# sebrahimi1988/dss-ml-at-scale

Measured on AMD Instinct MI355X. Metric: samples/sec, higher is better.
Workload: dtype bf16; 1 GPU; model=resnet18, global_batch=212, parallelism=dp1+hipgraph

## Files before the change

### mi355x_scale/ops/csrc/bindings.cpp

```cpp

#include <torch/extension.h>
#include <ATen/hip/HIPContext.h>
#include <hip/hip_runtime.h>

extern "C" void launch_normalize_u8_to_bf16(
    const uint8_t* in, void* out, const float* scale_dev,
    const float* shift_dev, long long n, hipStream_t stream);

void normalize_u8_to_bf16(torch::Tensor in, torch::Tensor out,
                          torch::Tensor scale, torch::Tensor shift) {
  TORCH_CHECK(in.is_cuda() && out.is_cuda(), "tensors must be on GPU");
  TORCH_CHECK(in.scalar_type() == torch::kUInt8, "input must be uint8");
  TORCH_CHECK(out.scalar_type() == torch::kBFloat16, "output must be bf16");
  TORCH_CHECK(in.is_contiguous(), "input must be contiguous (NHWC)");
  TORCH_CHECK(in.numel() == out.numel(), "element count mismatch");
  TORCH_CHECK(scale.is_cuda() && shift.is_cuda() && scale.numel() == 3 &&
                  shift.numel() == 3,
              "scale/shift must be 3-element device float tensors");
  TORCH_CHECK(scale.scalar_type() == torch::kFloat32 &&
              shift.scalar_type() == torch::kFloat32,
              "scale/shift must be float32");
  auto stream = at::cuda::getCurrentHIPStream();
  launch_normalize_u8_to_bf16(
      in.data_ptr<uint8_t>(), out.data_ptr(),
      scale.data_ptr<float>(), shift.data_ptr<float>(),
      (long long)in.numel(), stream.stream());
}

extern "C" void launch_groupfit_eval(
    const float* yT, const float* xc0, const float* xc1, const float* xc2,
    const float* pj0, const float* pj1, const float* pj2, const int* orders,
    float* mse, unsigned char* statusv,
    const float* b0, const float* b1, const float* b2,
    const float* w0, const float* w1, const float* w2,
    int T, long long G, int S, int C,
    int KX, hipStream_t stream);

extern "C" void launch_diff_center(const float* yT, float* wc, float* wm,
                                   int T, long long G, int S, int d,
                                   hipStream_t stream);

extern "C" void launch_exog_project_mfma(const float* P, const float* wc,
                                         float* beta, int n, long long G,
                                         int KX, hipStream_t stream);

extern "C" void launch_groupfit_final(
    const float* yT, const float* xc0, const float* xc1, const float* xc2,
    const float* pj0, const float* pj1, const float* pj2,
    const int* best_order, float* fitted, float* params,
    unsigned char* statusv,
    const float* b0, const float* b1, const float* b2,
    const float* w0, const float* w1, const float* w2,
    int T, long long G, int KX, hipStream_t stream);

extern "C" void launch_stem_conv_fwd(const void* x, const void* w, void* out,
                                     void* wp_scratch, float* partial,
                                     int Nb, int H, int W, int HO, int WO,
                                     hipStream_t stream, int phase_mask);
extern "C" int stem_fwd_stat_blocks(int Nb, int HO);
extern "C" void launch_stem_conv_wrw(const void* x, const void* dy,
                                     float* dw_f32, void* dw_bf16,
                                     int Nb, int H, int W, int HO, int WO,
                                     hipStream_t stream, int phase_mask);
extern "C" void launch_conv3x3_wrw(const void* x, const void* dy,
                                   float* part, void* dw_bf16,
                                   int Nb, int H, int W, int C,
                                   int chunks, hipStream_t stream,
                                   int phase_mask);
extern "C" int conv3x3_wrw_chunks(int Nb, int H, int C, int chunks_req);

static void _check_f32(const torch::Tensor& t, const char* name) {
  TORCH_CHECK(t.is_cuda() && t.scalar_type() == torch::kFloat32 &&
                  t.is_contiguous(),
              name, " must be contiguous f32 on GPU");
}

void groupfit_eval(torch::Tensor yT, torch::Tensor xc0, torch::Tensor xc1,
                   torch::Tensor xc2, torch::Tensor pj0, torch::Tensor pj1,
                   torch::Tensor pj2, torch::Tensor orders,
                   torch::Tensor mse, torch::Tensor status, int64_t S,
                   torch::Tensor b0, torch::Tensor b1, torch::Tensor b2,
                   torch::Tensor w0, torch::Tensor w1, torch::Tensor w2) {
  _check_f32(yT, "yT"); _check_f32(xc0, "xc0"); _check_f32(xc1, "xc1");
  _check_f32(xc2, "xc2"); _check_f32(pj0, "pj0"); _check_f32(pj1, "pj1");
  _check_f32(pj2, "pj2"); _check_f32(mse, "mse");
  TORCH_CHECK(orders.scalar_type() == torch::kInt32 && orders.is_cuda());
  TORCH_CHECK(status.scalar_type() == torch::kUInt8 && status.is_cuda());
  int T = yT.size(0);
  long long G = yT.size(1);
  int C = orders.size(0);
  TORCH_CHECK(S > 8 && S <= T, "need 8 < S <= T");
  TORCH_CHECK(mse.size(0) == C && mse.size(1) == G);
  auto stream = at::cuda::getCurrentHIPStream();
  auto fp = [](torch::Tensor& t) -> const float* {
    return t.numel() ? t.data_ptr<float>() : nullptr;
  };
  launch_groupfit_eval(
      yT.data_ptr<float>(), xc0.data_ptr<float>(), xc1.data_ptr<float>(),
      xc2.data_ptr<float>(), pj0.data_ptr<float>(), pj1.data_ptr<float>(),
      pj2.data_ptr<float>(), orders.data_ptr<int>(), mse.data_ptr<float>(),
      status.data_ptr<uint8_t>(),
      fp(b0), fp(b1), fp(b2), fp(w0), fp(w1), fp(w2),
      T, G, (int)S, C, (int)xc0.size(1),
      stream.stream());
}

void groupfit_final(torch::Tensor yT, torch::Tensor xc0, torch::Tensor xc1,
                    torch::Tensor xc2, torch::Tensor pj0, torch::Tensor pj1,
                    torch::Tensor pj2, torch::Tensor best_order,
                    torch::Tensor fitted, torch::Tensor params,
                    torch::Tensor status,
                    torch::Tensor b0, torch::Tensor b1, torch::Tensor b2,
                    torch::Tensor w0, torch::Tensor w1, torch::Tensor w2) {
  _check_f32(yT, "yT"); _check_f32(fitted, "fitted");
  _check_f32(params, "params");
  TORCH_CHECK(best_order.scalar_type() == torch::kInt32 &&
              best_order.is_cuda());
  int T = yT.size(0);
  long long G = yT.size(1);
  TORCH_CHECK(fitted.size(0) == T && fitted.size(1) == G);
  auto stream = at::cuda::getCurrentHIPStream();
  auto fp = [](torch::Tensor& t) -> const float* {
    return t.numel() ? t.data_ptr<float>() : nullptr;
  };
  launch_groupfit_final(
      yT.data_ptr<float>(), xc0.data_ptr<float>(), xc1.data_ptr<float>(),
      xc2.data_ptr<float>(), pj0.data_ptr<float>(), pj1.data_ptr<float>(),
      pj2.data_ptr<float>(), best_order.data_ptr<int>(),
      fitted.data_ptr<float>(), params.data_ptr<float>(),
      status.data_ptr<uint8_t>(),
      fp(b0), fp(b1), fp(b2), fp(w0), fp(w1), fp(w2),
      T, G, (int)xc0.size(1), stream.stream());
}

void diff_center(torch::Tensor yT, torch::Tensor wc, torch::Tensor wm,
                 int64_t S, int64_t d) {
  _check_f32(yT, "yT"); _check_f32(wc, "wc"); _check_f32(wm, "wm");
  auto stream = at::cuda::getCurrentHIPStream();
  launch_diff_center(yT.data_ptr<float>(), wc.data_ptr<float>(),
                     wm.data_ptr<float>(), yT.size(0), yT.size(1),
                     (int)S, (int)d, stream.stream());
}

void exog_project_mfma(torch::Tensor P, torch::Tensor wc,
                       torch::Tensor beta) {
  _check_f32(P, "P"); _check_f32(wc, "wc"); _check_f32(beta, "beta");
  TORCH_CHECK(P.size(1) == wc.size(0), "K mismatch");
  TORCH_CHECK(beta.size(0) == P.size(0) && beta.size(1) == wc.size(1));
  TORCH_CHECK(P.size(0) <= 16, "KX must fit one MFMA row tile");
  auto stream = at::cuda::getCurrentHIPStream();
  launch_exog_project_mfma(P.data_ptr<float>(), wc.data_ptr<float>(),
                           beta.data_ptr<float>(), P.size(1), wc.size(1),
                           P.size(0), stream.stream());
}


extern "C" int bn_reduce_blocks(long long rows, int C);
extern "C" void launch_bn_fwd_reduce(const void* x, float* partial,
                                     int nblocks, long long rows, int C,
                                     hipStream_t stream);
extern "C" void launch_bn_fwd_finalize(const float* partial, int nblocks,
                                       float* mean, float* invstd,
                                       float* running_mean,
                                       float* running_var, float momentum,
                                       float eps, long long rows, int C,
                                       int update_running,
                                       long long* num_batches_tracked,
                                       hipStream_t stream);
extern "C" void launch_bn_pool_bwd_reduce(
    const void* dp, const unsigned char* code, const void* x,
    const float* mean, const float* invstd, const float* weight,
    const float* bias, float* partial, int nblocks, int N, int H, int W,
    int Ho, int Wo, int C, hipStream_t stream);
extern "C" void launch_bn_pool_bwd_apply(
    const void* dp, const unsigned char* code, const void* x,
    const float* mean, const float* invstd, const float* bias,
    const float* k, void* dx, int N, int H, int W, int Ho, int Wo, int C,
    hipStream_t stream);
extern "C" void launch_bn_fwd_apply(const void* x, const void* res, void* y,
                                    const float* mean, const float* invstd,
                                    const float* weight, const float* bias,
                                    long long rows, int C, int relu,
                                    hipStream_t stream);
extern "C" void launch_bn_bwd_reduce(const void* dz, const void* y,
                                     const void* x, const float* mean,
                                     const float* invstd, float* partial,
                                     void* dym, int nblocks, long long rows,
                                     int C, int relu, hipStream_t stream);
extern "C" void launch_bn_bwd_reduce_join(const void* dz1, const void* dz2,
                                          const void* y, const void* x,
                                          const float* mean,
                                          const float* invstd,
                                          float* partial, void* dym,
                                          int nblocks, long long rows, int C,
                                          int relu, hipStream_t stream);
extern "C" void launch_bn_bwd_reduce_rm(const void* dz, const void* x,
                                        const float* mean,
                                        const float* invstd,
                                        const float* weight,
                                        const float* bias, float* partial,
                                        void* dym, int nblocks,
                                        long long rows, int C,
                                        hipStream_t stream);
extern "C" void launch_bn_bwd_apply_rm(const void* dz, const void* x,
                                       const float* mean,
                                       const float* invstd,
                                       const float* bias, const float* k,
                                       void* dx, long long rows, int C,
                                       hipStream_t stream);
extern "C" void launch_bn_bwd_apply_dym(const void* dym, const void* x,
                                        const float* mean,
                                        const float* invstd, const float* k,
                                        void* dx, long long rows, int C,
                                        hipStream_t stream);
extern "C" void launch_bn_bwd_finalize(const float* partial, int nblocks,
                                       const float* invstd,
// ... 322 lines not shown
  TORCH_CHECK(x.dim() == 4 && dp.dim() == 4, "x and dp must be 4-d");
  TORCH_CHECK(x.is_contiguous(at::MemoryFormat::ChannelsLast) &&
                  dp.is_contiguous(at::MemoryFormat::ChannelsLast),
              "x and dp must be channels_last");
  _PoolGeom g{(int)x.size(0), (int)x.size(1), (int)x.size(2),
              (int)x.size(3), (int)dp.size(2), (int)dp.size(3)};
  TORCH_CHECK(g.C % 8 == 0 && 256 % (g.C / 8) == 0, "bad C");
  TORCH_CHECK(dp.size(0) == g.N && dp.size(1) == g.C, "dp N/C mismatch");
  TORCH_CHECK(g.Ho == (g.H + 1) / 2 && g.Wo == (g.W + 1) / 2,
              "3x3 s2 p1 shape");
  TORCH_CHECK(code.numel() == dp.numel(), "code/dp size mismatch");
  TORCH_CHECK((int64_t)g.N * g.Ho * g.Wo < (int64_t(1) << 31),
              "N*Ho*Wo must be < 2^31");
  return g;
}

torch::Tensor bn_pool_bwd_reduce(torch::Tensor dp, torch::Tensor code,
                                 torch::Tensor x, torch::Tensor mean,
                                 torch::Tensor invstd, torch::Tensor weight,
                                 torch::Tensor bias) {
  _PoolGeom g = _check_bn_pool_bwd(dp, code, x);
  _check_f32(mean, "mean"); _check_f32(invstd, "invstd");
  _check_f32(weight, "weight"); _check_f32(bias, "bias");
  TORCH_CHECK(mean.numel() == g.C && invstd.numel() == g.C &&
                  weight.numel() == g.C && bias.numel() == g.C,
              "channel vectors must be [C]");
  int nb = bn_reduce_blocks((long long)g.N * g.Ho * g.Wo, g.C);
  auto partial = torch::empty(
      {(int64_t)nb * 2 * g.C},
      torch::TensorOptions().dtype(torch::kFloat32).device(x.device()));
  launch_bn_pool_bwd_reduce(dp.data_ptr(), code.data_ptr<uint8_t>(),
                            x.data_ptr(), mean.data_ptr<float>(),
                            invstd.data_ptr<float>(),
                            weight.data_ptr<float>(),
                            bias.data_ptr<float>(),
                            partial.data_ptr<float>(), nb, g.N, g.H, g.W,
                            g.Ho, g.Wo, g.C,
                            at::cuda::getCurrentHIPStream().stream());
  return partial;
}

void bn_pool_bwd_apply(torch::Tensor dp, torch::Tensor code, torch::Tensor x,
                       torch::Tensor mean, torch::Tensor invstd,
                       torch::Tensor bias, torch::Tensor k,
                       torch::Tensor dx) {
  _PoolGeom g = _check_bn_pool_bwd(dp, code, x);
  _check_bn_act(dx, "dx");
  _check_f32(mean, "mean"); _check_f32(invstd, "invstd");
  _check_f32(bias, "bias"); _check_f32(k, "k");
  TORCH_CHECK(mean.numel() == g.C && invstd.numel() == g.C &&
                  bias.numel() == g.C && k.numel() == 3 * g.C,
              "channel vectors must be [C], k [3C]");
  TORCH_CHECK(dx.sizes() == x.sizes() &&
                  dx.is_contiguous(at::MemoryFormat::ChannelsLast),
              "dx must match x (channels_last)");
  launch_bn_pool_bwd_apply(dp.data_ptr(), code.data_ptr<uint8_t>(),
                           x.data_ptr(), mean.data_ptr<float>(),
                           invstd.data_ptr<float>(), bias.data_ptr<float>(),
                           k.data_ptr<float>(), dx.data_ptr(), g.N, g.H,
                           g.W, g.Ho, g.Wo, g.C,
                           at::cuda::getCurrentHIPStream().stream());
}

extern "C" void launch_adam_step(float* p, const float* g, float* m,
                                 float* v, int* step, float lr, float beta1,
                                 float beta2, float eps, float weight_decay,
                                 long long n, hipStream_t stream);

void adam_step(torch::Tensor p, torch::Tensor g, torch::Tensor m,
               torch::Tensor v, torch::Tensor step, double lr, double beta1,
               double beta2, double eps, double weight_decay) {
  _check_f32(p, "p"); _check_f32(g, "g"); _check_f32(m, "m");
  _check_f32(v, "v");
  TORCH_CHECK(step.is_cuda() && step.scalar_type() == torch::kInt32 &&
                  step.numel() == 1,
              "step must be a 1-element int32 device tensor");
  long long n = p.numel();
  TORCH_CHECK(g.numel() == n && m.numel() == n && v.numel() == n,
              "flat buffer length mismatch");
  launch_adam_step(p.data_ptr<float>(), g.data_ptr<float>(),
                   m.data_ptr<float>(), v.data_ptr<float>(),
                   step.data_ptr<int>(), (float)lr, (float)beta1,
                   (float)beta2, (float)eps, (float)weight_decay, n,
                   at::cuda::getCurrentHIPStream().stream());
}

extern "C" void launch_adam_step_mixed(float* master, const void* gb,
                                       const float* gf, float* m, float* v,
                                       void* pb, int* step, float lr,
                                       float beta1, float beta2, float eps,
                                       float weight_decay, long long nb,
                                       long long n, hipStream_t stream);

void adam_step_mixed(torch::Tensor master, torch::Tensor gb,
                     torch::Tensor gf, torch::Tensor m, torch::Tensor v,
                     torch::Tensor pb, torch::Tensor step, double lr,
                     double beta1, double beta2, double eps,
                     double weight_decay) {
  _check_f32(master, "master"); _check_f32(m, "m"); _check_f32(v, "v");
  TORCH_CHECK(gb.scalar_type() == torch::kBFloat16 &&
              pb.scalar_type() == torch::kBFloat16, "gb/pb must be bf16");
  TORCH_CHECK(step.is_cuda() && step.scalar_type() == torch::kInt32 &&
              step.numel() == 1, "step must be int32[1] on device");
  long long n = master.numel();
  long long nb = gb.numel();
  TORCH_CHECK(pb.numel() == nb && gf.numel() == n - nb &&
              m.numel() == n && v.numel() == n, "buffer length mismatch");
  const float* gf_p = gf.numel() ? gf.data_ptr<float>() : nullptr;
  launch_adam_step_mixed(master.data_ptr<float>(), gb.data_ptr(), gf_p,
                         m.data_ptr<float>(), v.data_ptr<float>(),
                         pb.data_ptr(), step.data_ptr<int>(), (float)lr,
                         (float)beta1, (float)beta2, (float)eps,
                         (float)weight_decay, nb, n,
                         at::cuda::getCurrentHIPStream().stream());
}

int64_t stem_fwd_blocks(int64_t Nb, int64_t HO) {
  return stem_fwd_stat_blocks((int)Nb, (int)HO);
}

void stem_conv_fwd(torch::Tensor x, torch::Tensor w, torch::Tensor out,
                   torch::Tensor wp_scratch, int64_t phase_mask = 7,
                   c10::optional<torch::Tensor> partial = c10::nullopt) {
  TORCH_CHECK(x.is_cuda() && x.scalar_type() == torch::kBFloat16);
  TORCH_CHECK(w.is_cuda() && w.scalar_type() == torch::kBFloat16);
  TORCH_CHECK(out.is_cuda() && out.scalar_type() == torch::kBFloat16);
  int Nb = x.size(0), H = x.size(1), W = x.size(2);
  TORCH_CHECK(x.size(3) == 3 && out.size(3) == 64, "stem is 3->64");
  int HO = out.size(1), WO = out.size(2);
  TORCH_CHECK(WO <= 128, "stem kernel handles output rows up to 128 px");
  TORCH_CHECK(w.numel() == 64 * 7 * 7 * 3);
  TORCH_CHECK(wp_scratch.scalar_type() == torch::kBFloat16 &&
              wp_scratch.numel() == 64 * 160);
  TORCH_CHECK(x.is_contiguous() && out.is_contiguous() &&
                  out.size(0) == Nb && HO == (H - 1) / 2 + 1 &&
                  WO == (W - 1) / 2 + 1,
              "stem conv: dense NHWC x/out with 7x7 s2 p3 geometry");
  float* partial_p = nullptr;
  if (partial.has_value()) {
    const torch::Tensor& p = *partial;
    TORCH_CHECK(p.is_cuda() && p.scalar_type() == torch::kFloat32 &&
                    p.is_contiguous() &&
                    p.numel() == 2 * 64 * stem_fwd_blocks(Nb, HO),
                "partial must be fp32 [2*64*stem_fwd_blocks(N, HO)]");
    partial_p = p.data_ptr<float>();
  }
  launch_stem_conv_fwd(x.data_ptr(), w.data_ptr(), out.data_ptr(),
                       wp_scratch.data_ptr(), partial_p,
                       Nb, H, W, HO, WO,
                       at::cuda::getCurrentHIPStream().stream(),
                       (int)phase_mask);
}

void stem_conv_wrw(torch::Tensor x, torch::Tensor dy, torch::Tensor dw_f32,
                   torch::Tensor dw, int64_t phase_mask = 7) {
  TORCH_CHECK(x.is_cuda() && x.scalar_type() == torch::kBFloat16);
  TORCH_CHECK(dy.is_cuda() && dy.scalar_type() == torch::kBFloat16);
  TORCH_CHECK(dw_f32.scalar_type() == torch::kFloat32 &&
              dw_f32.numel() == 64 * 160);
  TORCH_CHECK(dw.scalar_type() == torch::kBFloat16 &&
              dw.numel() == 64 * 7 * 7 * 3);
  int Nb = x.size(0), H = x.size(1), W = x.size(2);
  int HO = dy.size(1), WO = dy.size(2);
  launch_stem_conv_wrw(x.data_ptr(), dy.data_ptr(),
                       dw_f32.data_ptr<float>(), dw.data_ptr(),
                       Nb, H, W, HO, WO,
                       at::cuda::getCurrentHIPStream().stream(),
                       (int)phase_mask);
}

void conv3x3_wrw(torch::Tensor x, torch::Tensor dy, torch::Tensor part,
                 torch::Tensor dw, int64_t phase_mask = 7,
                 int64_t chunks = 0) {
  TORCH_CHECK(x.is_cuda() && x.scalar_type() == torch::kBFloat16);
  TORCH_CHECK(dy.is_cuda() && dy.scalar_type() == torch::kBFloat16);
  int Nb = x.size(0), H = x.size(1), W = x.size(2), C = x.size(3);
  TORCH_CHECK(dy.size(1) == H && dy.size(2) == W && dy.size(3) == C,
              "same-shape 3x3 s1 conv only");
  TORCH_CHECK(C % 64 == 0 && C <= 2048, "C must be a multiple of 64");
  TORCH_CHECK(W >= 3 && W <= 64, "row length outside kernel bounds");
  const int nch = conv3x3_wrw_chunks(Nb, H, C, (int)chunks);
  TORCH_CHECK(part.scalar_type() == torch::kFloat32 &&
              part.numel() >= (long long)nch * C * 9 * C,
              "partial buffer too small for ", nch, " chunks");
  TORCH_CHECK(dw.scalar_type() == torch::kBFloat16 &&
              dw.numel() == (long long)C * 9 * C);
  launch_conv3x3_wrw(x.data_ptr(), dy.data_ptr(), part.data_ptr<float>(),
                     dw.data_ptr(), Nb, H, W, C, nch,
                     at::cuda::getCurrentHIPStream().stream(),
                     (int)phase_mask);
}

int64_t conv3x3_wrw_nchunks(int64_t Nb, int64_t H, int64_t C,
                            int64_t chunks) {
  return conv3x3_wrw_chunks((int)Nb, (int)H, (int)C, (int)chunks);
}

PYBIND11_MODULE(TORCH_EXTENSION_NAME, m) {
  m.def("conv3x3_wrw", &conv3x3_wrw,
        "MFMA 3x3/s1 CxC weight grad (fp32 accum, bf16 cast to view)",
        pybind11::arg("x"), pybind11::arg("dy"), pybind11::arg("part"),
        pybind11::arg("dw"), pybind11::arg("phase_mask") = 7,
        pybind11::arg("chunks") = 0);
  m.def("conv3x3_wrw_nchunks", &conv3x3_wrw_nchunks,
        "partial-buffer chunk count the wrw launcher will use");
  m.def("stem_conv_fwd", &stem_conv_fwd,
        "MFMA stem conv fwd (7x7 s2, 3->64, NHWC bf16)",
        pybind11::arg("x"), pybind11::arg("w"), pybind11::arg("out"),
        pybind11::arg("wp_scratch"), pybind11::arg("phase_mask") = 7,
        pybind11::arg("partial") = pybind11::none());
  m.def("stem_fwd_blocks", &stem_fwd_blocks,
        "block (= BN partial slot) count of the fused-statistics stem fwd");
  m.def("stem_conv_wrw", &stem_conv_wrw,
        "MFMA stem conv weight-grad (fp32 accum + bf16 cast)",
        pybind11::arg("x"), pybind11::arg("dy"), pybind11::arg("dw_f32"),
        pybind11::arg("dw"), pybind11::arg("phase_mask") = 7);
  m.def("normalize_u8_to_bf16", &normalize_u8_to_bf16,
        "fused uint8 NHWC -> normalized bf16 (same memory order)");
  m.def("groupfit_eval", &groupfit_eval,
        "batched per-group ARIMAX candidate evaluation (validation MSE)");
  m.def("groupfit_final", &groupfit_final,
        "batched per-group final fit (fitted values + params)");
  m.def("diff_center", &diff_center,
        "difference + per-group centering of the time-major panel");
  m.def("exog_project_mfma", &exog_project_mfma,
        "design-matrix GEMM beta = P @ Wc on f32 MFMA");
  m.def("bn_fwd_reduce", &bn_fwd_reduce);
  m.def("bn_fwd_finalize", &bn_fwd_finalize,
        "mean/invstd + running stats (+ optional int64 step counter)",
        pybind11::arg("partial"), pybind11::arg("mean"),
        pybind11::arg("invstd"), pybind11::arg("running_mean"),
        pybind11::arg("running_var"), pybind11::arg("momentum"),
        pybind11::arg("eps"), pybind11::arg("rows"), pybind11::arg("C"),
        pybind11::arg("update_running"),
        pybind11::arg("num_batches_tracked") = pybind11::none());
  m.def("bn_fwd_apply", &bn_fwd_apply);
  m.def("bn_bwd_reduce", &bn_bwd_reduce);
  m.def("bn_bwd_reduce_join", &bn_bwd_reduce_join);
  m.def("bn_bwd_reduce_rm", &bn_bwd_reduce_rm);
  m.def("bn_bwd_apply_rm", &bn_bwd_apply_rm);
  m.def("bn_bwd_finalize", &bn_bwd_finalize);
  m.def("bn_bwd_apply", &bn_bwd_apply);
  m.def("bn_bwd_apply_dym", &bn_bwd_apply_dym);
  m.def("adam_step", &adam_step,
        "fused flat Adam step (one kernel over p/g/m/v)");
  m.def("maxpool3x3s2_fwd", &maxpool3x3s2_fwd);
  m.def("bn_maxpool3x3s2_fwd", &bn_maxpool3x3s2_fwd);
  m.def("maxpool3x3s2_bwd", &maxpool3x3s2_bwd);
  m.def("bn_pool_bwd_reduce", &bn_pool_bwd_reduce,
        "stem BN bwd reduce with the max-unpool rebuilt in registers");
  m.def("bn_pool_bwd_apply", &bn_pool_bwd_apply,
        "stem BN bwd apply with the max-unpool rebuilt in registers");
  m.def("adam_step_mixed", &adam_step_mixed,
        "fused flat Adam with bf16 params/grads + fp32 master");
  m.def("arma_generate", &arma_generate,
        "batched ARMA(p,q) sample paths, one group per lane");
}
```

### mi355x_scale/ops/csrc/stemconv.hip

```cpp
#include <hip/hip_runtime.h>
#include <hip/hip_bf16.h>

#define KH 7
#define KW 7
#define CI 3
#define CO 64
#define KTAP (KH * KW * CI)
#define KPAD 160
#define KLDS 168
#define PXPAD 128
#define XTROW ((4 + 2 * PXPAD + KW + 4) * CI + 3)
#define XTOFF 12
#define STRIDE 2
#define PADDING 3

typedef __bf16 bf16;
typedef __attribute__((ext_vector_type(8))) __bf16 bf16x8;
typedef __attribute__((ext_vector_type(4))) __bf16 bf16x4;
typedef __attribute__((ext_vector_type(4))) float f32x4;

__device__ __forceinline__ void stage_band(
    const bf16* __restrict__ x, bf16* xt, int n, int ho, int H, int W,
    int tid, int nthreads, bool prime) {
  const int rowlen = W * CI;
// ... 201 lines not shown
          if (ih >= 0 && ih < H && c >= 0 && c < nch)
            v[u] = reinterpret_cast<const bf16x4*>(
                x + ((long long)n * H + ih) * rowlen)[c];
        }
      }
#pragma unroll
      for (int u = 0; u < STAGE_DEPTH; ++u) {
        const int i = base + tid + u * nthreads;
        if (i < total) reinterpret_cast<bf16x4*>(xt)[i] = v[u];
      }
    }
  } else {
    const int total = nrows_in * XTROW;
    for (int i = tid; i < total; i += nthreads) {
      const int r = i / XTROW, e = i - r * XTROW - XTOFF;
      const int ih = ih0 + r;
      bf16 v = (bf16)0.0f;
      if (ih >= 0 && ih < H && e >= 0 && e < rowlen)
        v = x[((long long)n * H + ih) * rowlen + e];
      xt[i] = v;
    }
  }
}

extern "C" __global__ __launch_bounds__(256, 3) void stem_conv_fwd_stats_kernel(
    const bf16* __restrict__ x,
    const bf16* __restrict__ wp,
    bf16* __restrict__ out,
    float* __restrict__ partial,
    int Nb, int H, int W, int HO, int WO, int nchunks, int phase_mask) {
  __shared__ __attribute__((aligned(16))) bf16 xt[FWD_BAND_ROWS * XTROW];
  __shared__ __attribute__((aligned(16))) bf16 ot[4 * 32 * OTROW];
  __shared__ __attribute__((aligned(16))) unsigned short ktab[4 * KPAD / 4];
  const int tid = threadIdx.x;
  const int wave = tid >> 6;
  const int lane = tid & 63;
  const int row16 = lane & 15;
  const int kgrp = lane >> 4;
  const int n = blockIdx.x / nchunks;
  const int ho0 = (blockIdx.x - n * nchunks) * FWD_ROWS;
  const int rows = min(FWD_ROWS, HO - ho0);

  bf16x8 bfrag[KPAD / 32][4];
#pragma unroll
  for (int kk = 0; kk < KPAD / 32; ++kk)
#pragma unroll
    for (int c = 0; c < 4; ++c)
      bfrag[kk][c] = *reinterpret_cast<const bf16x8*>(
          wp + (c * 16 + row16) * KPAD + kk * 32 + kgrp * 8);

  if (tid < 4 * KPAD / 4) {
    const int g = tid / (KPAD / 4), i = tid - g * (KPAD / 4);
    const int k = (i >> 3) * 32 + g * 8 + (i & 7);
    ktab[tid] = (unsigned short)(2 * koff_of(min(k, KTAP - 1)));
  }
  if (phase_mask & 1)
    stage_band_rows(x, xt, n, ho0 * STRIDE - PADDING,
                    rows * STRIDE + KH - STRIDE, H, W, tid, 256);
  __syncthreads();
  if (!(phase_mask & 4)) return;

  float ssum[4] = {0.f, 0.f, 0.f, 0.f}, ssq[4] = {0.f, 0.f, 0.f, 0.f};
  const int pxb0 = (wave * 32 + row16) * (STRIDE * CI);
  const int pxb1 = (wave * 32 + 16 + row16) * (STRIDE * CI);
  bf16* tw = ot + wave * 32 * OTROW;
#pragma unroll 1
  for (int rr = 0; rr < rows; ++rr) {
    const int rshift = rr * STRIDE * XTROW;
#pragma unroll 1
    for (int m = 0; m < 2; ++m) {
      f32x4 acc[4];
#pragma unroll
      for (int c = 0; c < 4; ++c) acc[c] = (f32x4)0.0f;
      const unsigned rb = 2u * (unsigned)(rshift + (m ? pxb1 : pxb0));
      const uint4* tp = reinterpret_cast<const uint4*>(ktab) + kgrp * 5;
      asm volatile("" : "+v"(tp));
#pragma unroll
      for (int kk = 0; kk < KPAD / 32; ++kk) {
        const uint4 t4 = tp[kk];
        const unsigned tk[4] = {t4.x, t4.y, t4.z, t4.w};
        bf16x8 f;
#pragma unroll
        for (int j = 0; j < 8; ++j) {
          const int k = kk * 32 + kgrp * 8 + j;
          const bool kz = (kk == KPAD / 32 - 1) && k >= KTAP;
          const unsigned pk = tk[j >> 1];
          const unsigned ob = ((j & 1) ? (pk >> 16) : (pk & 0xffffu)) + rb;
          f[j] = *reinterpret_cast<const bf16*>(
              reinterpret_cast<const char*>(xt) + (kz ? 0u : ob));
        }
#pragma unroll
        for (int c = 0; c < 4; ++c)
          acc[c] = __builtin_amdgcn_mfma_f32_16x16x32_bf16(
              f, bfrag[kk][c], acc[c], 0, 0, 0);
      }
#pragma unroll
      for (int r = 0; r < 4; ++r) {
        const int pxl = m * 16 + kgrp * 4 + r;
        const bool live = wave * 32 + pxl < WO;
#pragma unroll
        for (int c = 0; c < 4; ++c) {
          const bf16 v = (bf16)acc[c][r];
          tw[pxl * OTROW + c * 16 + row16] = v;
          const float f = live ? (float)v : 0.f;
          ssum[c] += f;
          ssq[c] += f * f;
        }
      }
    }
    __builtin_amdgcn_fence(__ATOMIC_RELEASE, "wavefront");
    __builtin_amdgcn_wave_barrier();
    __builtin_amdgcn_fence(__ATOMIC_ACQUIRE, "wavefront");
    const long long rowbase = ((long long)n * HO + ho0 + rr) * WO;
#pragma unroll
    for (int t = 0; t < 4; ++t) {
      const int v = lane + t * 64;
      const int pxl = v >> 3, j8 = (v & 7) * 8;
      const int px = wave * 32 + pxl;
      const bf16x8 val = *reinterpret_cast<const bf16x8*>(
          tw + pxl * OTROW + j8);
      if (px < WO)
        *reinterpret_cast<bf16x8*>(out + (rowbase + px) * CO + j8) = val;
    }
    __builtin_amdgcn_fence(__ATOMIC_RELEASE, "wavefront");
    __builtin_amdgcn_wave_barrier();
    __builtin_amdgcn_fence(__ATOMIC_ACQUIRE, "wavefront");
  }

#pragma unroll
  for (int c = 0; c < 4; ++c) {
    ssum[c] += __shfl_xor(ssum[c], 16, 64);
    ssum[c] += __shfl_xor(ssum[c], 32, 64);
    ssq[c] += __shfl_xor(ssq[c], 16, 64);
    ssq[c] += __shfl_xor(ssq[c], 32, 64);
  }
  float* red = reinterpret_cast<float*>(tw);
  if (kgrp == 0) {
#pragma unroll
    for (int c = 0; c < 4; ++c) {
      red[c * 16 + row16] = ssum[c];
      red[CO + c * 16 + row16] = ssq[c];
    }
  }
  __syncthreads();
  if (tid < 2 * CO) {
    float t = 0.f;
#pragma unroll
    for (int w = 0; w < 4; ++w)
      t += reinterpret_cast<const float*>(ot + w * 32 * OTROW)[tid];
    partial[(long long)tid * gridDim.x + blockIdx.x] = t;
  }
}

extern "C" __global__ __launch_bounds__(256) void stem_conv_wrw_kernel(
    const bf16* __restrict__ x,
    const bf16* __restrict__ dy,
    float* __restrict__ dw,
    int Nb, int H, int W, int HO, int WO, int rows_per_block,
    int phase_mask) {
  __shared__ bf16 xt[8 * XTROW];
  __shared__ bf16 Dy[2 * PXPAD * CO];
  const int tid = threadIdx.x;
  const int wave = tid >> 6;
  const int lane = tid & 63;
  const int row16 = lane & 15;
  const int kgrp = lane >> 4;
  const int nrows = Nb * HO;
  const int mw = (wave >> 1) * 2;
  const int cw = (wave & 1) * 5;
  const int row_limit = min((blockIdx.x + 1) * rows_per_block, nrows);
  const int nch = (WO * CO) >> 3;
  const bf16x8 zv = {(bf16)0.0f, (bf16)0.0f, (bf16)0.0f, (bf16)0.0f,
                     (bf16)0.0f, (bf16)0.0f, (bf16)0.0f, (bf16)0.0f};

  f32x4 acc[2][5];
#pragma unroll
  for (int m = 0; m < 2; ++m)
#pragma unroll
    for (int c = 0; c < 5; ++c) acc[m][c] = (f32x4)0.0f;

  int cur = 0;
  {
    const int row0 = blockIdx.x * rows_per_block;
    if (row0 < nrows) {
      const bf16x8* src = reinterpret_cast<const bf16x8*>(
          dy + (long long)row0 * WO * CO);
      bf16x8* d8 = reinterpret_cast<bf16x8*>(Dy);
      bf16x8 v[4];
#pragma unroll
      for (int u = 0; u < 4; ++u) {
        const int i = tid + u * 256;
        v[u] = (i < nch) ? src[i] : zv;
      }
#pragma unroll
      for (int u = 0; u < 4; ++u) d8[tid + u * 256] = v[u];
    }
  }

  for (int rr = 0; rr < rows_per_block; ++rr) {
    const int row = blockIdx.x * rows_per_block + rr;
    if (row >= nrows) break;
    const int n = row / HO;
    const int ho = row - n * HO;
    const bool prime = (rr == 0) || (ho == 0);
    __syncthreads();
    if (prime)
      for (int i = tid; i < 8 * XTROW; i += 256) xt[i] = (bf16)0.0f;
    __syncthreads();
    if (phase_mask & 1)
      stage_band_ring(x, xt, n, ho, H, W, tid, 256, prime);
    bf16x8 v[4];
    const bool have_next = (phase_mask & 2) && row + 1 < row_limit;
    if (have_next) {
      const bf16x8* src = reinterpret_cast<const bf16x8*>(
          dy + (long long)(row + 1) * WO * CO);
#pragma unroll
      for (int u = 0; u < 4; ++u) {
        const int i = tid + u * 256;
        v[u] = (i < nch) ? src[i] : zv;
      }
    }
    __syncthreads();
    if (phase_mask & 4) {
    } else {
      if (have_next) {
        bf16x8* d8 = reinterpret_cast<bf16x8*>(Dy + (cur ^ 1) * PXPAD * CO);
#pragma unroll
        for (int u = 0; u < 4; ++u) d8[tid + u * 256] = v[u];
        cur ^= 1;
      }
      continue;
    }

#pragma unroll
    for (int sl = 0; sl < 4; ++sl) {
      const int pxbase = sl * 32;
      bf16x8 afrag[2];
#pragma unroll
      for (int m = 0; m < 2; ++m) {
        bf16x8 f;
        const bf16* dycur = Dy + cur * PXPAD * CO;
#pragma unroll
        for (int j = 0; j < 8; ++j)
          f[j] = dycur[(pxbase + kgrp * 8 + j) * CO + (mw + m) * 16 + row16];
        afrag[m] = f;
      }
#pragma unroll
      for (int c = 0; c < 5; ++c) {
        const int k = (cw + c) * 16 + row16;
        const int kh = k / (KW * CI);
        const int r21 = k - kh * (KW * CI);
        const int ko = ((ho * STRIDE - PADDING + kh) & 7) * XTROW +
                       (XTOFF - PADDING * CI) + r21;
        const bool kz = k >= KTAP;
        bf16x8 bfr;
#pragma unroll
        for (int j = 0; j < 8; ++j)
          bfr[j] = kz ? (bf16)0.0f
                      : xt[ko + (pxbase + kgrp * 8 + j) * (STRIDE * CI)];
#pragma unroll
        for (int m = 0; m < 2; ++m)
          acc[m][c] = __builtin_amdgcn_mfma_f32_16x16x32_bf16(
              afrag[m], bfr, acc[m][c], 0, 0, 0);
      }
    }
    if (have_next) {
      bf16x8* d8 = reinterpret_cast<bf16x8*>(Dy + (cur ^ 1) * PXPAD * CO);
#pragma unroll
      for (int u = 0; u < 4; ++u) d8[tid + u * 256] = v[u];
      cur ^= 1;
    }
  }

#pragma unroll
  for (int m = 0; m < 2; ++m)
#pragma unroll
    for (int c = 0; c < 5; ++c)
#pragma unroll
      for (int r = 0; r < 4; ++r) {
        const int co = (mw + m) * 16 + kgrp * 4 + r;
        const int k = (cw + c) * 16 + row16;
        atomicAdd(&dw[co * KPAD + k], acc[m][c][r]);
      }
}

extern "C" __global__ __launch_bounds__(256) void stem_wrw_cast_kernel(
    const float* __restrict__ dw, bf16* __restrict__ out) {
  const int i = blockIdx.x * 256 + threadIdx.x;
  if (i < CO * KTAP) {
    const int co = i / KTAP, k = i - co * KTAP;
    out[i] = (bf16)dw[co * KPAD + k];
  }
}

extern "C" int stem_fwd_stat_blocks(int Nb, int HO) {
  return Nb * ((HO + FWD_ROWS - 1) / FWD_ROWS);
}

extern "C" void launch_stem_conv_fwd(const void* x, const void* w, void* out,
                                     void* wp_scratch, float* partial,
                                     int Nb, int H, int W, int HO, int WO,
                                     hipStream_t stream, int phase_mask) {
  hipLaunchKernelGGL(stem_pad_weights_kernel,
                     dim3((CO * KPAD + 255) / 256), dim3(256), 0, stream,
                     (const bf16*)w, (bf16*)wp_scratch);
  if (partial) {
    const int nchunks = (HO + FWD_ROWS - 1) / FWD_ROWS;
    hipLaunchKernelGGL(stem_conv_fwd_stats_kernel, dim3(Nb * nchunks),
                       dim3(256), 0, stream, (const bf16*)x,
                       (const bf16*)wp_scratch, (bf16*)out, partial,
                       Nb, H, W, HO, WO, nchunks, phase_mask);
    return;
  }
  hipLaunchKernelGGL(stem_conv_fwd_kernel, dim3(Nb * HO), dim3(256), 0,
                     stream, (const bf16*)x, (const bf16*)wp_scratch,
                     (bf16*)out, Nb, H, W, HO, WO, phase_mask);
}

extern "C" void launch_stem_conv_wrw(const void* x, const void* dy,
                                     float* dw_f32, void* dw_bf16,
                                     int Nb, int H, int W, int HO, int WO,
                                     hipStream_t stream,
                                     int phase_mask = 7) {
  const int nrows = Nb * HO;
  const int target_blocks = 768;
  const int rpb = (nrows + target_blocks - 1) / target_blocks;
  const int blocks = (nrows + rpb - 1) / rpb;
  hipMemsetAsync(dw_f32, 0, CO * KPAD * sizeof(float), stream);
  hipLaunchKernelGGL(stem_conv_wrw_kernel, dim3(blocks), dim3(256), 0,
                     stream, (const bf16*)x, (const bf16*)dy, dw_f32,
                     Nb, H, W, HO, WO, rpb, phase_mask);
  hipLaunchKernelGGL(stem_wrw_cast_kernel,
                     dim3((CO * KTAP + 255) / 256), dim3(256), 0, stream,
                     dw_f32, (bf16*)dw_bf16);
}
```

### mi355x_scale/ops/stemconv.py

```python
from __future__ import annotations

import os

import torch
import torch.nn as nn
import torch.nn.functional as F


def fused_stats_enabled() -> bool:
    return os.environ.get("MI355X_STEM_FUSED_STATS", "1") != "0"


def _stem_forward(x: torch.Tensor, weight: torch.Tensor, fused: bool):
    from . import _C
    N, C, H, W = x.shape
    HO = (H + 2 * 3 - 7) // 2 + 1
    WO = (W + 2 * 3 - 7) // 2 + 1
    out = torch.empty((N, 64, HO, WO), dtype=torch.bfloat16,
                      device=x.device,
                      memory_format=torch.channels_last)
    wp = torch.empty(64 * 160, dtype=torch.bfloat16, device=x.device)
    partial = None
    if fused:
        partial = torch.empty(2 * 64 * _C.stem_fwd_blocks(N, HO),
                              dtype=torch.float32, device=x.device)
    _C.stem_conv_fwd(x.permute(0, 2, 3, 1), weight.permute(0, 2, 3, 1),
                     out.permute(0, 2, 3, 1), wp, 7, partial)
    return out, partial


def _stem_backward(ctx, dy: torch.Tensor):
    from . import _C
    x, weight = ctx.saved_tensors
    if dy.dtype != torch.bfloat16:
        dy = dy.to(torch.bfloat16)
    dy = dy.contiguous(memory_format=torch.channels_last)
    dw = torch.empty_like(weight)
    scratch = torch.empty(64 * 160, dtype=torch.float32,
                          device=x.device)
    _C.stem_conv_wrw(x.permute(0, 2, 3, 1), dy.permute(0, 2, 3, 1),
                     scratch, dw.permute(0, 2, 3, 1))
    return None, dw


class _StemConvFn(torch.autograd.Function):
    @staticmethod
    def forward(ctx, x: torch.Tensor, weight: torch.Tensor):
        out, _ = _stem_forward(x, weight, fused_stats_enabled())
        ctx.save_for_backward(x, weight)
        return out

    @staticmethod
    def backward(ctx, dy: torch.Tensor):
        return _stem_backward(ctx, dy)


class _StemConvStatsFn(torch.autograd.Function):

    @staticmethod
    def forward(ctx, x: torch.Tensor, weight: torch.Tensor):
        out, partial = _stem_forward(x, weight, True)
        ctx.save_for_backward(x, weight)
        ctx.mark_non_differentiable(partial)
        ctx.set_materialize_grads(False)
        return out, partial

    @staticmethod
    def backward(ctx, dy, _dpartial):
        if dy is None:
            return None, None
        return _stem_backward(ctx, dy)


class StemConv2d(nn.Conv2d):

    def __init__(self):
        super().__init__(3, 64, 7, stride=2, padding=3, bias=False)

    def _hip_ok(self, x: torch.Tensor) -> bool:
        from . import HAVE_EXT
        return (HAVE_EXT and x.is_cuda
                and os.environ.get("MI355X_STEM_CONV", "1") == "1"
                and x.shape[-1] <= 262
                and x.dtype == torch.bfloat16
                and self.weight.dtype == torch.bfloat16
                and x.is_contiguous(memory_format=torch.channels_last)
                and self.weight.is_contiguous(
                    memory_format=torch.channels_last)
                and not x.requires_grad)

    def stats_ok(self, x: torch.Tensor) -> bool:
        return fused_stats_enabled() and self._hip_ok(x)

    def forward_with_stats(self, x: torch.Tensor):
        if self.stats_ok(x):
            return _StemConvStatsFn.apply(x, self.weight)
        return self.forward(x), None

    def forward(self, x: torch.Tensor) -> torch.Tensor:
        if self._hip_ok(x):
            return _StemConvFn.apply(x, self.weight)
        if x.is_cuda and torch.cuda.is_available():
            from . import HAVE_EXT, require_ext
            if HAVE_EXT is False and x.dtype == torch.bfloat16:
                require_ext()
        return F.conv2d(x, self.weight, None, self.stride, self.padding)
```

Measured before the change: 27170 samples/s.

## Rewrite stem conv weight-grad with LDS transpose reads and row-banded staging

Adds a new stem 7x7 weight-grad kernel that keeps a ring of input rows in LDS (duplicated at an odd offset for stride-2 parity) and uses ds_read_tr16 transposed reads to build MFMA fragments. It prefetches the next dy row and the next two input rows into registers while computing the current one. The old gather kernel stays available behind an env flag. The new kernel pads K to 176, so the scratch and cast kernel gain a remapped layout. The goal is cheaper fragment construction and less redundant input loading, at the cost of more LDS per block, which may limit occupancy.

```diff
diff --git a/mi355x_scale/ops/csrc/bindings.cpp b/mi355x_scale/ops/csrc/bindings.cpp
--- a/mi355x_scale/ops/csrc/bindings.cpp
+++ b/mi355x_scale/ops/csrc/bindings.cpp
@@ -2,6 +2,7 @@
 #include <torch/extension.h>
 #include <ATen/hip/HIPContext.h>
 #include <hip/hip_runtime.h>
+#include <cstdlib>
 
 extern "C" void launch_normalize_u8_to_bf16(
     const uint8_t* in, void* out, const float* scale_dev,
@@ -61,7 +62,9 @@
 extern "C" void launch_stem_conv_wrw(const void* x, const void* dy,
                                      float* dw_f32, void* dw_bf16,
                                      int Nb, int H, int W, int HO, int WO,
-                                     hipStream_t stream, int phase_mask);
+                                     hipStream_t stream, int phase_mask,
+                                     int tr);
+extern "C" int stem_wrw_scratch_elems();
 extern "C" void launch_conv3x3_wrw(const void* x, const void* dy,
                                    float* part, void* dw_bf16,
                                    int Nb, int H, int W, int C,
@@ -690,21 +693,36 @@
                        (int)phase_mask);
 }
 
+int64_t stem_wrw_scratch() { return stem_wrw_scratch_elems(); }
+
 void stem_conv_wrw(torch::Tensor x, torch::Tensor dy, torch::Tensor dw_f32,
-                   torch::Tensor dw, int64_t phase_mask = 7) {
+                   torch::Tensor dw, int64_t phase_mask = 7,
+                   int64_t tr = -1) {
   TORCH_CHECK(x.is_cuda() && x.scalar_type() == torch::kBFloat16);
   TORCH_CHECK(dy.is_cuda() && dy.scalar_type() == torch::kBFloat16);
-  TORCH_CHECK(dw_f32.scalar_type() == torch::kFloat32 &&
-              dw_f32.numel() == 64 * 160);
+  TORCH_CHECK(dw_f32.is_cuda() && dw_f32.scalar_type() == torch::kFloat32 &&
+                  dw_f32.is_contiguous() &&
+                  dw_f32.numel() == stem_wrw_scratch(),
+              "dw_f32 must be fp32 [stem_wrw_scratch()]");
   TORCH_CHECK(dw.scalar_type() == torch::kBFloat16 &&
               dw.numel() == 64 * 7 * 7 * 3);
   int Nb = x.size(0), H = x.size(1), W = x.size(2);
   int HO = dy.size(1), WO = dy.size(2);
+  TORCH_CHECK(x.size(3) == 3 && dy.size(3) == 64, "stem is 3->64");
+  TORCH_CHECK(WO <= 128, "stem kernel handles output rows up to 128 px");
+  TORCH_CHECK(x.is_contiguous() && dy.is_contiguous() &&
+                  dy.size(0) == Nb && HO == (H - 1) / 2 + 1 &&
+                  WO == (W - 1) / 2 + 1,
+              "stem conv: dense NHWC x/dy with 7x7 s2 p3 geometry");
+  if (tr < 0) {
+    const char* e = std::getenv("MI355X_STEM_WRW_TR");
+    tr = !(e && e[0] == '0' && e[1] == 0);
+  }
   launch_stem_conv_wrw(x.data_ptr(), dy.data_ptr(),
                        dw_f32.data_ptr<float>(), dw.data_ptr(),
                        Nb, H, W, HO, WO,
                        at::cuda::getCurrentHIPStream().stream(),
-                       (int)phase_mask);
+                       (int)phase_mask, tr ? 1 : 0);
 }
 
 void conv3x3_wrw(torch::Tensor x, torch::Tensor dy, torch::Tensor part,
@@ -752,7 +770,10 @@
   m.def("stem_conv_wrw", &stem_conv_wrw,
         "MFMA stem conv weight-grad (fp32 accum + bf16 cast)",
         pybind11::arg("x"), pybind11::arg("dy"), pybind11::arg("dw_f32"),
-        pybind11::arg("dw"), pybind11::arg("phase_mask") = 7);
+        pybind11::arg("dw"), pybind11::arg("phase_mask") = 7,
+        pybind11::arg("tr") = -1);
+  m.def("stem_wrw_scratch", &stem_wrw_scratch,
+        "fp32 element count of the stem weight-grad accumulation scratch");
   m.def("normalize_u8_to_bf16", &normalize_u8_to_bf16,
         "fused uint8 NHWC -> normalized bf16 (same memory order)");
   m.def("groupfit_eval", &groupfit_eval,
diff --git a/mi355x_scale/ops/csrc/stemconv.hip b/mi355x_scale/ops/csrc/stemconv.hip
--- a/mi355x_scale/ops/csrc/stemconv.hip
+++ b/mi355x_scale/ops/csrc/stemconv.hip
@@ -377,7 +377,7 @@
   }
 }
 
-extern "C" __global__ __launch_bounds__(256) void stem_conv_wrw_kernel(
+extern "C" __global__ __launch_bounds__(256) void stem_conv_wrw_gather_kernel(
     const bf16* __restrict__ x,
     const bf16* __restrict__ dy,
     float* __restrict__ dw,
@@ -509,12 +509,262 @@
       }
 }
 
+#define TRK 24
+#define KPADT 176
+#define NKT (KPADT / 16)
+#define DYROW 80
+#define XTIMG (8 * XTROW)
+#define XTODD (XTIMG + 2)
+
+typedef __attribute__((ext_vector_type(2))) __bf16 bf16x2;
+typedef __attribute__((ext_vector_type(4))) short s16x4;
+typedef __attribute__((ext_vector_type(8))) short s16x8;
+
+__device__ __forceinline__ bf16x8 tr_frag(const bf16* p0, const bf16* p1) {
+  typedef __attribute__((address_space(3))) s16x4 lds_s16x4;
+  const s16x4 lo = __builtin_amdgcn_ds_read_tr16_b64_v4i16((lds_s16x4*)p0);
+  const s16x4 hi = __builtin_amdgcn_ds_read_tr16_b64_v4i16((lds_s16x4*)p1);
+  const s16x8 v = __builtin_shufflevector(lo, hi, 0, 1, 2, 3, 4, 5, 6, 7);
+  return __builtin_bit_cast(bf16x8, v);
+}
+
+__device__ __forceinline__ void band_put(bf16* xt, int slot, int c,
+                                         bf16x4 v) {
+  bf16* e = xt + slot * XTROW + XTOFF + 4 * c;
+  *reinterpret_cast<bf16x4*>(e) = v;
+  const bf16x2 lo = {v[0], v[1]}, hi = {v[2], v[3]};
+  *reinterpret_cast<bf16x2*>(e + XTODD) = lo;
+  *reinterpret_cast<bf16x2*>(e + XTODD + 2) = hi;
+}
+
+__device__ __forceinline__ void wrw_stage_rows(
+    const bf16* __restrict__ x, bf16* xt, int n, int ho, int rfirst,
+    int H, int W, int tid) {
+  const int rowlen = W * CI;
+  const int ih0 = ho * STRIDE - PADDING;
+  if ((rowlen & 3) == 0) {
+    const int nch = rowlen >> 2;
+    const int total = (KH - rfirst) * nch;
+    const bf16x4 z = {(bf16)0.0f, (bf16)0.0f, (bf16)0.0f, (bf16)0.0f};
+    for (int base = 0; base < total; base += 256 * 4) {
+      bf16x4 v[4];
+      int ss[4], cc[4];
+#pragma unroll
+      for (int u = 0; u < 4; ++u) {
+        const int i = base + tid + u * 256;
+        v[u] = z;
+        ss[u] = -1;
+        if (i < total) {
+          const int r = i / nch, c = i - r * nch;
+          const int ih = ih0 + rfirst + r;
+          ss[u] = ih & 7; cc[u] = c;
+          if (ih >= 0 && ih < H)
+            v[u] = reinterpret_cast<const bf16x4*>(
+                x + ((long long)n * H + ih) * rowlen)[c];
+        }
+      }
+#pragma unroll
+      for (int u = 0; u < 4; ++u)
+        if (ss[u] >= 0) band_put(xt, ss[u], cc[u], v[u]);
+    }
+  } else {
+    for (int r = rfirst; r < KH; ++r) {
+      const int ih = ih0 + r;
+      const bool in = ih >= 0 && ih < H;
+      const bf16* src = x + ((long long)n * H + (in ? ih : 0)) * rowlen;
+      bf16* dst = xt + (ih & 7) * XTROW + XTOFF;
+      for (int i = tid; i < rowlen; i += 256) {
+        const bf16 v = in ? src[i] : (bf16)0.0f;
+        dst[i] = v;
+        dst[i + XTODD] = v;
+      }
+    }
+  }
+}
+
+extern "C" __global__ __launch_bounds__(256, 3) void stem_conv_wrw_kernel(
+    const bf16* __restrict__ x,
+    const bf16* __restrict__ dy,
+    float* __restrict__ dw,
+    int Nb, int H, int W, int HO, int WO, int rows_per_block,
+    int phase_mask) {
+  __shared__ __attribute__((aligned(16))) bf16 xt[2 * XTIMG];
+  __shared__ __attribute__((aligned(16))) bf16 Dy[PXPAD * DYROW];
+  const int tid = threadIdx.x;
+  const int wave = __builtin_amdgcn_readfirstlane(tid >> 6);
+  const int lane = tid & 63;
+  const int l16 = lane & 15;
+  const int kgrp = lane >> 4;
+  const int q = l16 >> 2, p = l16 & 3;
+  const int nrows = Nb * HO;
+  const int mw = (wave >> 1) * 2;
+  const int cw = (wave & 1) * 6;
+  const int nk = min(6, NKT - cw);
+  const int row0 = blockIdx.x * rows_per_block;
+  const int row_limit = min(row0 + rows_per_block, nrows);
+  if (row0 >= nrows) return;
+  const int rowlen = W * CI;
+  const bool vec = (rowlen & 3) == 0;
+  const int nchx = rowlen >> 2;
+  const int nch = (WO * CO) >> 3;
+  const bf16x8 zv = {(bf16)0.0f, (bf16)0.0f, (bf16)0.0f, (bf16)0.0f,
+                     (bf16)0.0f, (bf16)0.0f, (bf16)0.0f, (bf16)0.0f};
+  const bf16x4 zx = {(bf16)0.0f, (bf16)0.0f, (bf16)0.0f, (bf16)0.0f};
+
+  f32x4 acc[2][6];
+#pragma unroll
+  for (int m = 0; m < 2; ++m)
+#pragma unroll
+    for (int c = 0; c < 6; ++c) acc[m][c] = (f32x4)0.0f;
+
+  int aoff[2], boffpx[2];
+#pragma unroll
+  for (int t = 0; t < 2; ++t) {
+    const int par = (kgrp + t) & 1;
+    const int px = 8 * kgrp + par + 2 * q;
+    aoff[t] = px * DYROW + mw * 16 + 4 * p;
+    boffpx[t] = par * XTODD + px * (STRIDE * CI);
+  }
+  int khc[6], rc[6];
+#pragma unroll
+  for (int c = 0; c < 6; ++c) {
+    const int kq = (cw + c) * 16 + 4 * p;
+    khc[c] = kq / TRK;
+    rc[c] = kq - khc[c] * TRK;
+  }
+
+  for (int i = tid; i < 2 * XTIMG / 8; i += 256)
+    reinterpret_cast<bf16x8*>(xt)[i] = zv;
+  {
+    const bf16x8* src = reinterpret_cast<const bf16x8*>(
+        dy + (long long)row0 * WO * CO);
+    bf16x8 v[4];
+#pragma unroll
+    for (int u = 0; u < 4; ++u) {
+      const int i = tid + u * 256;
+      v[u] = (i < nch) ? src[i] : zv;
+    }
+#pragma unroll
+    for (int u = 0; u < 4; ++u) {
+      const int i = tid + u * 256;
+      *reinterpret_cast<bf16x8*>(Dy + (i >> 3) * DYROW + (i & 7) * 8) = v[u];
+    }
+  }
+  __syncthreads();
+  if (phase_mask & 1)
+    wrw_stage_rows(x, xt, row0 / HO, row0 % HO, 0, H, W, tid);
+  __syncthreads();
+
+  int n = row0 / HO;
+  int ho = row0 - n * HO;
+  for (int row = row0; row < row_limit; ++row) {
+    const bool have_next = row + 1 < row_limit;
+    const bool next_same = have_next && ho + 1 < HO;
+    bf16x8 v[4];
+    bf16x4 bv[2];
+    if (have_next && (phase_mask & 2)) {
+      const bf16x8* src = reinterpret_cast<const bf16x8*>(
+          dy + (long long)(row + 1) * WO * CO);
+#pragma unroll
+      for (int u = 0; u < 4; ++u) {
+        const int i = tid + u * 256;
+        v[u] = (i < nch) ? src[i] : zv;
+      }
+    }
+    const int ihn = (ho + 1) * STRIDE - PADDING + (KH - STRIDE);
+    if (next_same && vec && (phase_mask & 1)) {
+#pragma unroll
+      for (int u = 0; u < 2; ++u) {
+        const int i = tid + u * 256;
+        const int r = i >= nchx ? 1 : 0;
+        const int c = i - r * nchx;
+        bv[u] = zx;
+        if (c < nchx && ihn + r < H)
+          bv[u] = reinterpret_cast<const bf16x4*>(
+              x + ((long long)n * H + ihn + r) * rowlen)[c];
+      }
+    }
+
+    if (phase_mask & 4) {
+      const int ih0 = ho * STRIDE - PADDING;
+      int boff[6];
+#pragma unroll
+      for (int c = 0; c < 6; ++c)
+        boff[c] = ((ih0 + khc[c]) & 7) * XTROW + rc[c];
+#pragma unroll
+      for (int sl = 0; sl < 4; ++sl) {
+        if (sl * 32 >= WO) break;
+        bf16x8 af[2];
+#pragma unroll
+        for (int m = 0; m < 2; ++m)
+          af[m] = tr_frag(Dy + aoff[0] + sl * 32 * DYROW + m * 16,
+                          Dy + aoff[1] + sl * 32 * DYROW + m * 16);
+#pragma unroll
+        for (int c = 0; c < 6; ++c) {
+          if (c < nk) {
+            const int so = sl * 32 * STRIDE * CI;
+            const bf16x8 bfr = tr_frag(xt + boff[c] + boffpx[0] + so,
+                                       xt + boff[c] + boffpx[1] + so);
+#pragma unroll
+            for (int m = 0; m < 2; ++m)
+              acc[m][c] = __builtin_amdgcn_mfma_f32_16x16x32_bf16(
+                  af[m], bfr, acc[m][c], 0, 0, 0);
+          }
+        }
+      }
+    }
+    if (!have_next) break;
+
+    __syncthreads();
+    if (phase_mask & 2) {
+#pragma unroll
+      for (int u = 0; u < 4; ++u) {
+        const int i = tid + u * 256;
+        *reinterpret_cast<bf16x8*>(Dy + (i >> 3) * DYROW + (i & 7) * 8) =
+            v[u];
+      }
+    }
+    if (phase_mask & 1) {
+      if (!next_same) {
+        wrw_stage_rows(x, xt, n + 1, 0, 0, H, W, tid);
+      } else if (!vec) {
+        wrw_stage_rows(x, xt, n, ho + 1, KH - STRIDE, H, W, tid);
+      } else {
+#pragma unroll
+        for (int u = 0; u < 2; ++u) {
+          const int i = tid + u * 256;
+          const int r = i >= nchx ? 1 : 0;
+          const int c = i - r * nchx;
+          if (c < nchx) band_put(xt, (ihn + r) & 7, c, bv[u]);
+        }
+      }
+    }
+    __syncthreads();
+    if (++ho == HO) { ho = 0; ++n; }
+  }
+
+#pragma unroll
+  for (int m = 0; m < 2; ++m)
+#pragma unroll
+    for (int c = 0; c < 6; ++c)
+      if (c < nk) {
+#pragma unroll
+        for (int r = 0; r < 4; ++r) {
+          const int co = (mw + m) * 16 + kgrp * 4 + r;
+          const int k = (cw + c) * 16 + l16;
+          atomicAdd(&dw[co * KPADT + k], acc[m][c][r]);
+        }
+      }
+}
+
 extern "C" __global__ __launch_bounds__(256) void stem_wrw_cast_kernel(
-    const float* __restrict__ dw, bf16* __restrict__ out) {
+    const float* __restrict__ dw, bf16* __restrict__ out, int tr) {
   const int i = blockIdx.x * 256 + threadIdx.x;
   if (i < CO * KTAP) {
     const int co = i / KTAP, k = i - co * KTAP;
-    out[i] = (bf16)dw[co * KPAD + k];
+    const int kh = k / (KW * CI);
+    out[i] = (bf16)(tr ? dw[co * KPADT + k + kh * (TRK - KW * CI) + 3]
+                       : dw[co * KPAD + k]);
   }
 }
 
@@ -546,16 +796,23 @@
                                      float* dw_f32, void* dw_bf16,
                                      int Nb, int H, int W, int HO, int WO,
                                      hipStream_t stream,
-                                     int phase_mask = 7) {
+                                     int phase_mask, int tr) {
   const int nrows = Nb * HO;
   const int target_blocks = 768;
   const int rpb = (nrows + target_blocks - 1) / target_blocks;
   const int blocks = (nrows + rpb - 1) / rpb;
-  hipMemsetAsync(dw_f32, 0, CO * KPAD * sizeof(float), stream);
-  hipLaunchKernelGGL(stem_conv_wrw_kernel, dim3(blocks), dim3(256), 0,
-                     stream, (const bf16*)x, (const bf16*)dy, dw_f32,
-                     Nb, H, W, HO, WO, rpb, phase_mask);
+  (void)hipMemsetAsync(dw_f32, 0, CO * KPADT * sizeof(float), stream);
+  if (tr)
+    hipLaunchKernelGGL(stem_conv_wrw_kernel, dim3(blocks), dim3(256), 0,
+                       stream, (const bf16*)x, (const bf16*)dy, dw_f32,
+                       Nb, H, W, HO, WO, rpb, phase_mask);
+  else
+    hipLaunchKernelGGL(stem_conv_wrw_gather_kernel, dim3(blocks), dim3(256),
+                       0, stream, (const bf16*)x, (const bf16*)dy, dw_f32,
+                       Nb, H, W, HO, WO, rpb, phase_mask);
   hipLaunchKernelGGL(stem_wrw_cast_kernel,
                      dim3((CO * KTAP + 255) / 256), dim3(256), 0, stream,
-                     dw_f32, (bf16*)dw_bf16);
-}
+                     dw_f32, (bf16*)dw_bf16, tr);
+}
+
+extern "C" int stem_wrw_scratch_elems() { return CO * KPADT; }
diff --git a/mi355x_scale/ops/stemconv.py b/mi355x_scale/ops/stemconv.py
--- a/mi355x_scale/ops/stemconv.py
+++ b/mi355x_scale/ops/stemconv.py
@@ -36,7 +36,7 @@
         dy = dy.to(torch.bfloat16)
     dy = dy.contiguous(memory_format=torch.channels_last)
     dw = torch.empty_like(weight)
-    scratch = torch.empty(64 * 160, dtype=torch.float32,
+    scratch = torch.empty(_C.stem_wrw_scratch(), dtype=torch.float32,
                           device=x.device)
     _C.stem_conv_wrw(x.permute(0, 2, 3, 1), dy.permute(0, 2, 3, 1),
                      scratch, dw.permute(0, 2, 3, 1))
@@ -81,7 +81,7 @@
         from . import HAVE_EXT
         return (HAVE_EXT and x.is_cuda
                 and os.environ.get("MI355X_STEM_CONV", "1") == "1"
-                and x.shape[-1] <= 262
+                and (x.shape[-1] - 1) // 2 + 1 <= 128
                 and x.dtype == torch.bfloat16
                 and self.weight.dtype == torch.bfloat16
                 and x.is_contiguous(memory_format=torch.channels_last)
```

New measurement: 27660 samples/s (median of 6 runs). +1.8%, better.
